# quan-dao/practical-collab-perception

Hardware: AMD Instinct MI355X
Metric: frames/sec (60k-pt cloud, 6 agents) (higher is better)
Workload: dtype f32

## Files before the change

### include/pcp_hip.h

```cpp
#ifndef PCP_HIP_H
#define PCP_HIP_H

#include <stddef.h>
#include <stdint.h>

#ifdef __cplusplus
extern "C" {
#endif

#define PCP_ABI_VERSION 1

enum {
  PCP_OK = 0,
  PCP_ERR_ARG = 1,
  PCP_ERR_WORKSPACE = 2,
  PCP_ERR_LAUNCH = 3,
  PCP_ERR_UNSUPPORTED = 4
};

int pcp_abi_version(void);
const char *pcp_status_string(int status);

enum {
  PCP_OPT_PFN_CROWD = 0,
  PCP_OPT_PFN_CROWD_BLOCKS = 1,
  PCP_OPT_PFN_WPS = 2,
  PCP_OPT_WINO4C_NW = 3,
  PCP_OPT_MP_TH16_MIN = 4,
  PCP_OPT_MP_DIAG = 5,
  PCP_OPT_VOX_AGGREGATE = 6,
  PCP_OPT_CONV_S2_FORM = 7,
  PCP_OPT_GTS_PASTE_FORM = 8,
  PCP_OPT_COUNT = 9
};
int pcp_set_option(int32_t option, int64_t value);
int64_t pcp_get_option(int32_t option);

typedef struct {
  float min_x, min_y, min_z;
  float voxel_x, voxel_y, voxel_z;
  int32_t nx, ny;
  int32_t batch_size;
} pcp_grid_t;

#define PCP_VOX_COUNTERS 4

size_t pcp_voxelize_workspace_bytes(const pcp_grid_t *grid, int64_t max_points);

int pcp_voxelize(const float *points, int64_t n, int32_t row_stride, const pcp_grid_t *grid,
                 void *workspace, size_t workspace_bytes,
                 int32_t *voxel_coords, int64_t *unq_inv, int32_t *unq_cnt, int32_t *counters, void *stream);
int pcp_voxelize_cells_ready(const float *points, int64_t n, int32_t row_stride, const pcp_grid_t *grid,
                             void *workspace, size_t workspace_bytes,
                             int32_t *voxel_coords, int32_t *unq_cnt, int32_t *counters, void *stream);

int pcp_voxelize_sort_pillar_rows(const pcp_grid_t *grid, void *workspace, int64_t n, void *stream);
int pcp_voxelize_row_order(const pcp_grid_t *grid, const void *workspace, int64_t n, int32_t *order, int32_t *cursor_scratch,
                           void *stream);

int pcp_pfn_scatter(const float *points, int64_t n, int32_t row_stride, int32_t num_raw, const pcp_grid_t *grid,
                    const void *workspace, const float *w0, const float *b0, const float *w1, const float *b1,
                    float *pillar_features, float *canvas, void *stream);

#define PCP_ROWS_CELLS_READY 1
#define PCP_ROWS_BUCKET_ORDER 2
size_t pcp_pillarise_rows_workspace_bytes(const pcp_grid_t *grid, int64_t max_points, int32_t num_raw);
int pcp_pillarise_rows(const float *points, int64_t n, int32_t row_stride, int32_t num_raw, const pcp_grid_t *grid,
                       void *workspace, size_t workspace_bytes, int32_t *voxel_coords, int64_t *unq_inv, int32_t *unq_cnt,
                       int32_t *counters, int32_t flags, void *stream);
int pcp_pfn_rows(const pcp_grid_t *grid, const void *workspace, int64_t n, int32_t num_raw, const float *w0, const float *b0,
                 const float *w1, const float *b1, float *pillar_features, float *canvas, void *stream);
int pcp_pillar_index_export(const pcp_grid_t *grid, const void *workspace, int64_t n, int32_t num_raw, int32_t *voxel_coords,
                            int32_t *row_rank, int32_t *slot_rank, int32_t *slot_canvas_row, int32_t *counters, void *stream);

#define PCP_PFN_ABSOLUTE_XYZ 1u
#define PCP_PFN_WITH_DISTANCE 2u
int pcp_pfn_features(const float *points, int64_t n, int32_t row_stride, int32_t num_raw, uint32_t flags, const pcp_grid_t *grid,
                     const void *vox_workspace, int32_t fw, float *fbuf, int32_t *slot_pillar, void *stream);
int pcp_pfn_cat_pillar_max(const float *y, int32_t ld_y, const float *pillar_max, int32_t ld_max, const int32_t *slot_pillar, int64_t rows,
                           int32_t c, float *out, int32_t ld_out, void *stream);

int pcp_canvas_clear(const pcp_grid_t *grid, const void *workspace, int64_t n, float *canvas, void *stream);
int pcp_fill_zero(void *ptr, size_t bytes, void *stream);

typedef struct {
  int32_t batch, in_h, in_w;
// ... 72 lines not shown
  int32_t batch, h, w, ld;
  int32_t num_class;
  int32_t ch_center, ch_z, ch_dim, ch_rot, ch_hm;
  int32_t k;
  float stride;
  float voxel_x, voxel_y, min_x, min_y;
  float limit[6];
  int32_t use_score_thresh;
  float score_thresh;
  int32_t activated;
} pcp_decode_t;

size_t pcp_decode_workspace_bytes(const pcp_decode_t *desc);
int pcp_centerhead_decode(const pcp_decode_t *desc, const float *head, void *workspace, size_t workspace_bytes,
                          float *boxes, float *scores, int32_t *labels, int32_t *cell, int32_t *count, void *stream);

#define PCP_DET_MAX_HEADS 8
typedef struct {
  const float *boxes;
  const float *scores;
  const int32_t *labels;
  const int32_t *keep;
  const int32_t *keep_count;
  const int32_t *class_map;
  int32_t k, keep_max;
} pcp_det_head_t;
int pcp_gather_detections(const pcp_det_head_t *heads, int32_t n_heads, int32_t batch, int32_t out_max, float *out_boxes,
                          float *out_scores, int64_t *out_labels, int32_t *out_count, void *stream);

size_t pcp_nms_workspace_bytes(int32_t n_max, int32_t batch);
int pcp_nms_rotated(const float *boxes, const float *scores, int32_t batch, int32_t n_max, const int32_t *n_dev,
                    float thresh, int32_t pre_max, int32_t post_max, void *workspace, size_t workspace_bytes,
                    int32_t *keep, int32_t *keep_count, void *stream);
int pcp_nms_normal(const float *boxes, const float *scores, int32_t batch, int32_t n_max, const int32_t *n_dev,
                   float thresh, int32_t pre_max, int32_t post_max, void *workspace, size_t workspace_bytes,
                   int32_t *keep, int32_t *keep_count, void *stream);
int pcp_boxes_bev_pairwise(const float *a, int32_t na, const float *b, int32_t nb, int32_t mode, float *out,
                           void *stream);

int pcp_warp_nearest(const float *src, float *dst, int32_t h, int32_t w, int32_t c, int32_t ld_src, int32_t ld_dst,
                     const float *theta_host, int32_t accumulate, void *stream);
int pcp_warp_nearest_batch(const float *const *src_host, float *const *dst_host, const float *theta_host, int32_t n_jobs, int32_t h,
                           int32_t w, int32_t c, int32_t ld_src, int32_t ld_dst, int32_t accumulate, void *stream);
int pcp_warp_nearest_batch_dev(const float *const *src_host, float *const *dst_host, const float *theta_dev, int32_t n_jobs, int32_t h,
                               int32_t w, int32_t c, int32_t ld_src, int32_t ld_dst, int32_t accumulate, void *stream);
int pcp_softmax_fuse(const float *const *maps_host, int32_t n_agents, const float *weights, int32_t ld_w, int64_t pixels,
                     int32_t c, int32_t ld_map, int32_t ld_out, float *out, void *stream);
int pcp_disco_weight_fuse(const float *const *maps_host, int32_t n_maps, int32_t c, int32_t ld_map, int64_t pixels,
                          const float *w1, const float *b1, const float *w2, const float *b2, const float *w3, const float *b3,
                          float *out, int32_t ld_out, float *logits, int32_t ld_w, void *stream);
int pcp_disco_weight_fuse_live(const float *const *maps_host, int32_t n_maps, int32_t c, int32_t ld_map, int64_t pixels,
                               const float *w1, const float *b1, const float *w2, const float *b2, const float *w3, const float *b3,
                               float *out, int32_t ld_out, const int32_t *live_index_host, const int32_t *live, void *stream);


int pcp_bev_sample_bilinear(const float *bev, int32_t batch, int32_t h, int32_t w, int32_t c, int32_t ld_bev,
                            const float *points, int64_t n, int32_t row_stride, float min_x, float min_y, float pix_x,
                            float pix_y, const uint8_t *row_mask, float *out, int32_t ld_out, void *stream);
int pcp_hunter_point_head(const float *bev, int32_t batch, int32_t h, int32_t w, int32_t c, int32_t ld_bev,
                          const float *points, int64_t n, int32_t row_stride, float min_x, float min_y, float pix_x,
                          float pix_y, const float *w1, const float *b1, const float *w2, const float *b2, const float *wh,
                          const float *bh, int32_t hidden, int32_t n_out, float *pf, int32_t ld_pf, float *head,
                          void *stream);
int pcp_hunter_point_head_ex(const float *bev, int32_t batch, int32_t h, int32_t w, int32_t c, int32_t ld_bev, float *points, int64_t n,
                             int32_t row_stride, float min_x, float min_y, float pix_x, float pix_y, const float *w1, const float *b1,
                             const float *w2, const float *b2, const float *wh, const float *bh, int32_t hidden, int32_t n_out, float *pf,
                             int32_t ld_pf, float *head, const int32_t *order, const int32_t *order_count, int32_t apply_flow,
                             float flow_thresh, uint8_t *dyn_mask, void *stream);
size_t pcp_bev_scatter_mean_workspace_bytes(int32_t batch, int32_t h, int32_t w, int64_t n);
int pcp_bev_scatter_mean(const float *points, int64_t n, int32_t row_stride, const float *feat, int32_t ld_feat,
                         int32_t c, int32_t batch, int32_t h, int32_t w, float min_x, float min_y, float pix_x,
                         float pix_y, void *workspace, size_t workspace_bytes, float *out, int32_t ld_out, void *stream);
int pcp_hunter_apply_flow(float *points, int64_t n, int32_t row_stride, const float *head, int32_t ld_head, float thresh,
                          uint8_t *row_mask, void *stream);

int pcp_select_transform_points(const float *points, int64_t n, int32_t row_stride, int32_t agent_col, float agent,
                                int32_t batch, const float *poses_host, const uint8_t *present_host, float *out,
                                int32_t out_batch_offset, void *stream);
int pcp_column_id_mask(const float *points, int64_t n, int32_t row_stride, int32_t col, uint64_t *out2, void *stream);
int pcp_column_id_counts(const float *points, int64_t n, int32_t row_stride, int32_t col, uint64_t *out66, void *stream);

int pcp_agent_frame_live(const float *points, int64_t n, int32_t row_stride, int32_t agent_col, int32_t batch, int32_t *live,
                         void *stream);
int pcp_zero_maps_unless(float *maps, int64_t map_elems, int32_t n_maps, const int32_t *flag_index_host, const int32_t *live,
                         void *stream);
size_t pcp_select_transform_compact_workspace_bytes(int64_t n, int32_t n_slots);
int pcp_select_transform_compact(const float *points, int64_t n, int32_t row_stride, int32_t agent_col, int32_t n_slots,
                                 const float *agents_host, int32_t batch, const float *poses_host, const uint8_t *present_host,
                                 float *out, int64_t out_rows, void *workspace, size_t workspace_bytes, int32_t *slot_start,
                                 const pcp_grid_t *vox_grid, void *vox_workspace, size_t vox_workspace_bytes, void *stream);
int pcp_select_transform_compact_dev(const float *points, int64_t n, int32_t row_stride, int32_t agent_col, int32_t n_slots,
                                     const float *agents_host, int32_t batch, const float *poses_dev, const uint8_t *present_dev,
                                     float *out, int64_t out_rows, void *workspace, size_t workspace_bytes, int32_t *slot_start,
                                     const pcp_grid_t *vox_grid, void *vox_workspace, size_t vox_workspace_bytes, void *stream);

int pcp_points_in_boxes(const float *boxes, int32_t batch, int32_t n_boxes, int32_t box_stride, const float *points, int32_t n_points,
                        int32_t point_stride, int32_t *box_idx, void *stream);
size_t pcp_hunter_foreground_workspace_bytes(int64_t n);
int pcp_hunter_foreground_rows(const float *points, int64_t n, int32_t row_stride, const float *head, int32_t ld_head, float thresh_bg,
                               void *workspace, size_t workspace_bytes, float *rows, int32_t *row_batch, int32_t *count, void *stream);
int pcp_modar_ingest(const float *modar, int32_t n_modar, const float *foreground, int32_t n_foreground, int32_t foreground_cols,
                     const double *target_se3_lidar_host, float max_sweep_idx, float *rows, void *stream);

size_t pcp_modar_ingest_batched_workspace_bytes(int32_t groups, int64_t max_foreground);
int pcp_modar_ingest_batched(const float *det_boxes, const float *det_scores, const int64_t *det_labels, const int32_t *det_count,
                             int32_t groups, int32_t det_max, const float *foreground, int32_t foreground_cols,
// ... 111 lines not shown
```

### practical-collab-perception_amd/csrc/abi.hip

```cpp
#include "pcp_common.h"

extern "C" int pcp_abi_version(void) { return PCP_ABI_VERSION; }

extern "C" const char *pcp_status_string(int status) {
  switch (status) {
    case PCP_OK: return "ok";
    case PCP_ERR_ARG: return "bad argument";
    case PCP_ERR_WORKSPACE: return "workspace too small";
    case PCP_ERR_LAUNCH: return "kernel launch failed";
    case PCP_ERR_UNSUPPORTED: return "unsupported shape for this build";
    default: return "unknown status";
  }
}

#include <atomic>

namespace {
std::atomic<long long> g_option[PCP_OPT_COUNT] = {{-1}, {-1}, {-1}, {-1}, {-1}, {-1}, {-1}, {-1}, {-1}};
static_assert(PCP_OPT_COUNT == 9, "one initialiser per option");
constexpr int MAX_DEVICES = 64;
std::atomic<int> g_cus[MAX_DEVICES];
}

extern "C" int pcp_set_option(int32_t option, int64_t value) {
  if (option < 0 || option >= PCP_OPT_COUNT) return PCP_ERR_ARG;
  g_option[option].store(value < 0 ? -1 : (long long)value, std::memory_order_relaxed);
  return PCP_OK;
}

extern "C" int64_t pcp_get_option(int32_t option) {
  if (option < 0 || option >= PCP_OPT_COUNT) return -1;
  return g_option[option].load(std::memory_order_relaxed);
}

long long pcp_option(int option, long long builtin) {
  const long long v = g_option[option].load(std::memory_order_relaxed);
  return v < 0 ? builtin : v;
}

int pcp_current_device_cus() {
  int dev = 0;
  if (hipGetDevice(&dev) != hipSuccess || dev < 0 || dev >= MAX_DEVICES) return 256;
  int v = g_cus[dev].load(std::memory_order_relaxed);
  if (v > 0) return v;
  if (hipDeviceGetAttribute(&v, hipDeviceAttributeMultiprocessorCount, dev) != hipSuccess || v <= 0) v = 256;
  g_cus[dev].store(v, std::memory_order_relaxed);
  return v;
}
```

### practical-collab-perception_amd/csrc/fusion.hip

```cpp
#include "pcp_common.h"

#pragma clang fp contract(off)

namespace {

struct Theta { float t[6]; };

__device__ __forceinline__ float base_coord(int i, int n) {
  if (n <= 1) return 0.f;
  float step = 2.0f / (float)(n - 1);
  float v = (i < n / 2) ? (-1.0f + step * (float)i) : (1.0f - step * (float)(n - 1 - i));
  return v * (float)(n - 1) / (float)n;
}

template <typename T> struct Map4;
template <> struct Map4<float> {
  static __device__ __forceinline__ float4 ld(const float *p) { return *reinterpret_cast<const float4 *>(p); }
  static __device__ __forceinline__ void st(float *p, const float4 &v) { *reinterpret_cast<float4 *>(p) = v; }
};
template <> struct Map4<__bf16> {
  typedef __bf16 b4 __attribute__((ext_vector_type(4)));
  static __device__ __forceinline__ float4 ld(const __bf16 *p) {
    const b4 v = *reinterpret_cast<const b4 *>(p);
    return make_float4((float)v[0], (float)v[1], (float)v[2], (float)v[3]);
  }
  static __device__ __forceinline__ void st(__bf16 *p, const float4 &v) {
    b4 o;
    o[0] = (__bf16)v.x; o[1] = (__bf16)v.y; o[2] = (__bf16)v.z; o[3] = (__bf16)v.w;
    *reinterpret_cast<b4 *>(p) = o;
  }
};

template <typename ST, typename DT>
__global__ void k_warp_nearest(const ST *__restrict__ src, DT *__restrict__ dst, int h, int w, int c4, int ld_src,
                               int ld_dst, Theta th, int accumulate) {
  long long t = (long long)blockIdx.x * blockDim.x + threadIdx.x;
  long long total = (long long)h * w * c4;
  if (t >= total) return;
  int q = (int)(t % c4);
  int pix = (int)(t / c4);
  int oy = pix / w, ox = pix % w;
  float xn = base_coord(ox, w), yn = base_coord(oy, h);
  float gx = xn * th.t[0] + yn * th.t[1] + th.t[2];
  float gy = xn * th.t[3] + yn * th.t[4] + th.t[5];
  float fx = (gx + 1.0f) * ((float)w / 2.0f) - 0.5f;
  float fy = (gy + 1.0f) * ((float)h / 2.0f) - 0.5f;
  float rx = nearbyintf(fx), ry = nearbyintf(fy);
  float4 v = make_float4(0.f, 0.f, 0.f, 0.f);
  if (rx >= 0.f && rx <= (float)(w - 1) && ry >= 0.f && ry <= (float)(h - 1)) {
    int sx = (int)rx, sy = (int)ry;
    v = Map4<ST>::ld(src + ((long long)sy * w + sx) * ld_src + q * 4);
  }
  DT *o = dst + (long long)pix * ld_dst + q * 4;
  if (accumulate) {
    float4 cur = Map4<DT>::ld(o);
    v.x += cur.x; v.y += cur.y; v.z += cur.z; v.w += cur.w;
  }
  Map4<DT>::st(o, v);
}

constexpr int WARP_MAX_JOBS = 32;
struct WarpJobs {
  const float *src[WARP_MAX_JOBS];
  float *dst[WARP_MAX_JOBS];
  Theta th[WARP_MAX_JOBS];
};

__global__ void k_warp_nearest_batch(WarpJobs jobs, int h, int w, int c4, int ld_src, int ld_dst, int accumulate, const float *__restrict__ theta_dev,
                                     int theta_first) {
  const int j = blockIdx.y;
  const float *__restrict__ src = jobs.src[j];
  float *__restrict__ dst = jobs.dst[j];
  Theta th = jobs.th[j];
  if (theta_dev) {
#pragma unroll
    for (int i = 0; i < 6; i++) th.t[i] = theta_dev[(theta_first + j) * 6 + i];
  }
  long long t = (long long)blockIdx.x * blockDim.x + threadIdx.x;
  long long total = (long long)h * w * c4;
  if (t >= total) return;
  int q = (int)(t % c4);
  int pix = (int)(t / c4);
  int oy = pix / w, ox = pix % w;
  float xn = base_coord(ox, w), yn = base_coord(oy, h);
  float gx = xn * th.t[0] + yn * th.t[1] + th.t[2];
  float gy = xn * th.t[3] + yn * th.t[4] + th.t[5];
  float fx = (gx + 1.0f) * ((float)w / 2.0f) - 0.5f;
  float fy = (gy + 1.0f) * ((float)h / 2.0f) - 0.5f;
  float rx = nearbyintf(fx), ry = nearbyintf(fy);
  float4 v = make_float4(0.f, 0.f, 0.f, 0.f);
  if (rx >= 0.f && rx <= (float)(w - 1) && ry >= 0.f && ry <= (float)(h - 1)) {
    int sx = (int)rx, sy = (int)ry;
    v = *reinterpret_cast<const float4 *>(src + ((long long)sy * w + sx) * ld_src + q * 4);
  }
  float4 *o = reinterpret_cast<float4 *>(dst + (long long)pix * ld_dst + q * 4);
  if (accumulate) {
    float4 cur = *o;
    v.x += cur.x; v.y += cur.y; v.z += cur.z; v.w += cur.w;
  }
  *o = v;
}

constexpr int MAX_AGENTS = 16;
struct MapPtrs { const float *p[MAX_AGENTS]; };
struct VMapPtrs { const void *p[MAX_AGENTS]; };

template <typename MT>
__global__ void k_softmax_fuse(VMapPtrs maps, int n_agents, const float *__restrict__ weights, int ld_w, long long pixels,
                               int c4, int ld_map, int ld_out, float *__restrict__ out) {
  long long t = (long long)blockIdx.x * blockDim.x + threadIdx.x;
  if (t >= pixels * c4) return;
  int q = (int)(t % c4);
  long long pix = t / c4;
  float wv[MAX_AGENTS];
  float mx = -INFINITY;
#pragma unroll
  for (int a = 0; a < MAX_AGENTS; a++)
    if (a < n_agents) {
      wv[a] = weights[pix * ld_w + a];
      mx = fmaxf(mx, wv[a]);
    }
  float den = 0.f;
#pragma unroll
  for (int a = 0; a < MAX_AGENTS; a++)
    if (a < n_agents) {
      wv[a] = expf(wv[a] - mx);
      den += wv[a];
    }
  float4 acc = make_float4(0.f, 0.f, 0.f, 0.f);
#pragma unroll
  for (int a = 0; a < MAX_AGENTS; a++)
    if (a < n_agents) {
      float s = wv[a] / den;
      float4 m = Map4<MT>::ld(reinterpret_cast<const MT *>(maps.p[a]) + pix * ld_map + q * 4);
      acc.x += m.x * s; acc.y += m.y * s; acc.z += m.z * s; acc.w += m.w * s;
    }
  *reinterpret_cast<float4 *>(out + pix * ld_out + q * 4) = acc;
}

}

extern "C" int pcp_warp_nearest(const float *src, float *dst, int32_t h, int32_t w, int32_t c, int32_t ld_src, int32_t ld_dst,
                                const float *theta_host, int32_t accumulate, void *stream_) {
  if (!src || !dst || !theta_host || h <= 0 || w <= 0 || c <= 0 || (c & 3) || (ld_src & 3) || (ld_dst & 3)) return PCP_ERR_ARG;
  if (src == dst) return PCP_ERR_ARG;
  Theta th;
  for (int i = 0; i < 6; i++) th.t[i] = theta_host[i];
// ... 53 lines not shown

extern "C" int pcp_mp_warp_nearest(const void *src, int32_t src_dtype, void *dst, int32_t dst_dtype, int32_t h, int32_t w, int32_t c,
                                   int32_t ld_src, int32_t ld_dst, const float *theta_host, int32_t accumulate, void *stream_) {
  if (!src || !dst || !theta_host || h <= 0 || w <= 0 || c <= 0 || (c & 3) || (ld_src & 3) || (ld_dst & 3)) return PCP_ERR_ARG;
  if (src == dst || (src_dtype | dst_dtype) & ~1) return PCP_ERR_ARG;
  Theta th;
  for (int i = 0; i < 6; i++) th.t[i] = theta_host[i];
  const long long total = (long long)h * w * (c / 4);
  const dim3 grid((unsigned)((total + 255) / 256));
  hipStream_t st = (hipStream_t)stream_;
#define PCP_WARP(ST, DT) hipLaunchKernelGGL((k_warp_nearest<ST, DT>), grid, dim3(256), 0, st, (const ST *)src, (DT *)dst, h, w, c / 4, ld_src, ld_dst, th, accumulate)
  if (src_dtype == 1) { if (dst_dtype == 1) PCP_WARP(__bf16, __bf16); else PCP_WARP(__bf16, float); }
  else { if (dst_dtype == 1) PCP_WARP(float, __bf16); else PCP_WARP(float, float); }
#undef PCP_WARP
  PCP_CHECK_LAUNCH();
  return PCP_OK;
}

extern "C" int pcp_mp_softmax_fuse(const void *const *maps_host, int32_t map_dtype, int32_t n_agents, const float *weights, int32_t ld_w,
                                   int64_t pixels, int32_t c, int32_t ld_map, int32_t ld_out, float *out, void *stream_) {
  if (!maps_host || !weights || !out || n_agents <= 0 || n_agents > MAX_AGENTS || pixels <= 0 || c <= 0 || (c & 3) ||
      (ld_map & 3) || (ld_out & 3) || ld_w < n_agents || (map_dtype & ~1))
    return PCP_ERR_ARG;
  VMapPtrs mp;
  for (int a = 0; a < MAX_AGENTS; a++) mp.p[a] = a < n_agents ? maps_host[a] : nullptr;
  const long long total = pixels * (c / 4);
  const dim3 grid((unsigned)((total + 255) / 256));
  if (map_dtype == 1)
    hipLaunchKernelGGL((k_softmax_fuse<__bf16>), grid, dim3(256), 0, (hipStream_t)stream_, mp, n_agents, weights, ld_w, (long long)pixels, c / 4,
                       ld_map, ld_out, out);
  else
    hipLaunchKernelGGL((k_softmax_fuse<float>), grid, dim3(256), 0, (hipStream_t)stream_, mp, n_agents, weights, ld_w, (long long)pixels, c / 4,
                       ld_map, ld_out, out);
  PCP_CHECK_LAUNCH();
  return PCP_OK;
}


namespace {

constexpr int WF_PX = 64;
constexpr int WF_C = 128;
constexpr int WF_H1 = 64, WF_H2 = 16;
constexpr int WF_H1_LD = 68;

struct WfParams {
  MapPtrs maps;
  int n_maps, ld_map, ld_out, ld_w;
  long long pixels;
  const float *w1, *b1, *w2, *b2, *w3, *b3;
  float *out, *logits;
  const int *live;
  int live_idx[MAX_AGENTS];
};

}

#pragma clang fp contract(on)
namespace {
}

namespace {

__global__ __launch_bounds__(256, 2) void k_weight_fuse(WfParams p) {
  __shared__ __attribute__((aligned(16))) float h1[WF_PX * WF_H1_LD];
  __shared__ float h2[WF_PX][WF_H2 + 1];
  __shared__ float lg[MAX_AGENTS][WF_PX];
  const int tid = threadIdx.x, lane = tid & 63;
  const int wave = __builtin_amdgcn_readfirstlane(tid >> 6);
  const int rt = wave >> 1, ct = wave & 1;
  const int r = lane & 31, h = lane >> 5;
  f32x4 wb[16];
  const float *w1_row = p.w1 + (long long)(ct * 32 + r) * (2 * WF_C) + 4 * h;
#pragma unroll
  for (int j = 0; j < 16; j++) wb[j] = *reinterpret_cast<const f32x4 *>(w1_row + WF_C + 8 * j);
  const float bias1 = p.b1[ct * 32 + r];
  const long long n_tiles = (p.pixels + WF_PX - 1) / WF_PX;
  for (long long tile = blockIdx.x; tile < n_tiles; tile += gridDim.x) {
    const long long px0 = tile * WF_PX;
    long long prow = px0 + rt * 32 + r;
    if (prow >= p.pixels) prow = p.pixels - 1;
    f32x16 acc_e;
#pragma unroll
    for (int e = 0; e < 16; e++) acc_e[e] = 0.f;
    {
      const float *src = p.maps.p[0] + prow * p.ld_map + 4 * h;
#pragma unroll
      for (int j = 0; j < 16; j++) {
        const f32x4 a = *reinterpret_cast<const f32x4 *>(src + 8 * j);
        const f32x4 w = *reinterpret_cast<const f32x4 *>(w1_row + 8 * j);
        acc_e = mfma32(a.x, w.x, acc_e);
        acc_e = mfma32(a.y, w.y, acc_e);
        acc_e = mfma32(a.z, w.z, acc_e);
        acc_e = mfma32(a.w, w.w, acc_e);
      }
    }
    for (int a_i = 0; a_i < p.n_maps; a_i++) {
      f32x16 acc = acc_e;
      const float *src = p.maps.p[a_i] + prow * p.ld_map + 4 * h;
#pragma unroll
      for (int j = 0; j < 16; j++) {
        const f32x4 a = *reinterpret_cast<const f32x4 *>(src + 8 * j);
        acc = mfma32(a.x, wb[j].x, acc);
        acc = mfma32(a.y, wb[j].y, acc);
        acc = mfma32(a.z, wb[j].z, acc);
        acc = mfma32(a.w, wb[j].w, acc);
      }
#pragma unroll
      for (int e = 0; e < 16; e++) {
        const int row = rt * 32 + (e & 3) + 8 * (e >> 2) + 4 * h;
        h1[row * WF_H1_LD + ct * 32 + r] = fmaxf(acc[e] + bias1, 0.f);
      }
      __syncthreads();
      {
        const int px = lane, og = wave;
        float o[4];
#pragma unroll
        for (int i = 0; i < 4; i++) o[i] = p.b2[og * 4 + i];
        const float *xr = &h1[px * WF_H1_LD];
#pragma unroll
        for (int k4 = 0; k4 < WF_H1 / 4; k4++) {
          const f32x4 x = *reinterpret_cast<const f32x4 *>(xr + 4 * k4);
#pragma unroll
          for (int i = 0; i < 4; i++) {
            const float *wr = p.w2 + (og * 4 + i) * WF_H1 + 4 * k4;
            o[i] = fmaf(wr[0], x.x, o[i]);
            o[i] = fmaf(wr[1], x.y, o[i]);
            o[i] = fmaf(wr[2], x.z, o[i]);
            o[i] = fmaf(wr[3], x.w, o[i]);
          }
        }
#pragma unroll
        for (int i = 0; i < 4; i++) h2[px][og * 4 + i] = fmaxf(o[i], 0.f);
      }
      __syncthreads();
      if (tid < WF_PX) {
        float l = p.b3[0];
#pragma unroll
        for (int k = 0; k < WF_H2; k++) l = fmaf(p.w3[k], h2[tid][k], l);
        l = fmaxf(l, 0.f);
        if (p.live && p.live_idx[a_i] >= 0 && p.live[p.live_idx[a_i]] == 0) l = -INFINITY;
        lg[a_i][tid] = l;
        if (p.logits && px0 + tid < p.pixels) p.logits[(px0 + tid) * p.ld_w + a_i] = l;
      }
    }
    __syncthreads();
    if (tid < WF_PX) {
      float mx = -INFINITY;
      for (int a_i = 0; a_i < p.n_maps; a_i++) mx = fmaxf(mx, lg[a_i][tid]);
      float den = 0.f;
      for (int a_i = 0; a_i < p.n_maps; a_i++) {
        const float e = expf(lg[a_i][tid] - mx);
        lg[a_i][tid] = e;
        den += e;
      }
      for (int a_i = 0; a_i < p.n_maps; a_i++) lg[a_i][tid] = lg[a_i][tid] / den;
    }
    __syncthreads();
    {
#pragma clang fp contract(off)
      constexpr int WF_Q = WF_PX * (WF_C / 4) / 256;
      float4 facc[WF_Q];
#pragma unroll
      for (int i = 0; i < WF_Q; i++) facc[i] = make_float4(0.f, 0.f, 0.f, 0.f);
      for (int a_i = 0; a_i < p.n_maps; a_i++) {
        float4 m[WF_Q];
        float sv[WF_Q];
#pragma unroll
        for (int i = 0; i < WF_Q; i++) {
          const int idx = i * 256 + tid;
          const int px = idx >> 5, q = idx & 31;
          long long pp = px0 + px;
          if (pp >= p.pixels) pp = p.pixels - 1;
          m[i] = *reinterpret_cast<const float4 *>(p.maps.p[a_i] + pp * p.ld_map + q * 4);
          sv[i] = lg[a_i][px];
        }
#pragma unroll
        for (int i = 0; i < WF_Q; i++) {
          facc[i].x += m[i].x * sv[i]; facc[i].y += m[i].y * sv[i]; facc[i].z += m[i].z * sv[i]; facc[i].w += m[i].w * sv[i];
        }
      }
#pragma unroll
      for (int i = 0; i < WF_Q; i++) {
        const int idx = i * 256 + tid;
        const int px = idx >> 5, q = idx & 31;
        if (px0 + px < p.pixels) *reinterpret_cast<float4 *>(p.out + (px0 + px) * p.ld_out + q * 4) = facc[i];
      }
    }
    __syncthreads();
  }
}

}

static int disco_weight_fuse_impl(const float *const *maps_host, int32_t n_maps, int32_t c, int32_t ld_map, int64_t pixels,
                                  const float *w1, const float *b1, const float *w2, const float *b2, const float *w3, const float *b3,
                                  float *out, int32_t ld_out, float *logits, int32_t ld_w, const int32_t *live_index_host, const int32_t *live,
                                  void *stream_) {
  if (!maps_host || !w1 || !b1 || !w2 || !b2 || !w3 || !b3 || !out || n_maps <= 0 || n_maps > MAX_AGENTS || pixels <= 0) return PCP_ERR_ARG;
  if (c != WF_C) return PCP_ERR_UNSUPPORTED;
  if ((ld_map & 3) || (ld_out & 3) || ld_map < c || ld_out < c || (logits && ld_w < n_maps)) return PCP_ERR_ARG;
  if ((((uintptr_t)w1) & 15) || (((uintptr_t)out) & 15)) return PCP_ERR_ARG;
  WfParams p;
  for (int a = 0; a < MAX_AGENTS; a++) {
    p.maps.p[a] = a < n_maps ? maps_host[a] : nullptr;
    if (a < n_maps && (!maps_host[a] || (((uintptr_t)maps_host[a]) & 15))) return PCP_ERR_ARG;
  }
  p.n_maps = n_maps; p.ld_map = ld_map; p.ld_out = ld_out; p.ld_w = ld_w; p.pixels = pixels;
  p.w1 = w1; p.b1 = b1; p.w2 = w2; p.b2 = b2; p.w3 = w3; p.b3 = b3; p.out = out; p.logits = logits;
  p.live = live_index_host ? live : nullptr;
  for (int a = 0; a < MAX_AGENTS; a++) p.live_idx[a] = (live_index_host && a < n_maps) ? live_index_host[a] : -1;
  const long long n_tiles = (pixels + WF_PX - 1) / WF_PX;
  const unsigned blocks = (unsigned)(n_tiles < 512 ? n_tiles : 512);
  hipLaunchKernelGGL(k_weight_fuse, dim3(blocks), dim3(256), 0, (hipStream_t)stream_, p);
  PCP_CHECK_LAUNCH();
  return PCP_OK;
}

extern "C" int pcp_disco_weight_fuse(const float *const *maps_host, int32_t n_maps, int32_t c, int32_t ld_map, int64_t pixels,
                                     const float *w1, const float *b1, const float *w2, const float *b2, const float *w3, const float *b3,
                                     float *out, int32_t ld_out, float *logits, int32_t ld_w, void *stream_) {
  return disco_weight_fuse_impl(maps_host, n_maps, c, ld_map, pixels, w1, b1, w2, b2, w3, b3, out, ld_out, logits, ld_w, nullptr, nullptr, stream_);
}

extern "C" int pcp_disco_weight_fuse_live(const float *const *maps_host, int32_t n_maps, int32_t c, int32_t ld_map, int64_t pixels,
                                          const float *w1, const float *b1, const float *w2, const float *b2, const float *w3, const float *b3,
                                          float *out, int32_t ld_out, const int32_t *live_index_host, const int32_t *live, void *stream_) {
  if (!live_index_host || !live) return PCP_ERR_ARG;
  return disco_weight_fuse_impl(maps_host, n_maps, c, ld_map, pixels, w1, b1, w2, b2, w3, b3, out, ld_out, nullptr, 0, live_index_host, live, stream_);
}
```

### practical-collab-perception_amd/pcdet/models/bev_layers/v2x_fusion_disco.py

```python
import os

import numpy as np
import torch
import torch.nn as nn

from pcp_amd import fusion_host, lib, ops

from ..convnet import pack_conv_module
from ..packed import PackedModule, train_tape


class PixelWeightedFusionSoftmax(nn.Module):

    def __init__(self, channel):
        super().__init__()
        self.conv1_1 = nn.Conv2d(channel * 2, 64, kernel_size=1, stride=1, padding=0)
        self.bn1_1 = nn.BatchNorm2d(64)
        self.conv1_2 = nn.Conv2d(64, 16, kernel_size=1, stride=1, padding=0)
        self.bn1_2 = nn.BatchNorm2d(16)
        self.conv1_4 = nn.Conv2d(16, 1, kernel_size=1, stride=1, padding=0)


def transform_bev_img(dst_se3_src, bev_in_src, pc_range_min, pix_size):
    assert bev_in_src.dim() == 3
# ... 36 lines not shown
                    d1=pack_conv_module(self.decompressor[3], None, relu=False),
                    wf=self._fold_weightor())

    fused_weightor = os.environ.get('PCP_DISCO_FUSED_WEIGHTOR', '1') != '0'

    def _fold_weightor(self):
        from ..convnet import _fold
        pw = self.pixel_weightor
        w1, b1 = _fold(pw.conv1_1, pw.bn1_1, 0)
        w2, b2 = _fold(pw.conv1_2, pw.bn1_2, 0)
        w3, b3 = _fold(pw.conv1_4, None, 0)
        f = lambda t: t.reshape(t.shape[0], -1).float().contiguous()
        return dict(w1=f(w1), b1=b1.float().contiguous(), w2=f(w2), b2=b2.float().contiguous(), w3=f(w3).reshape(-1).contiguous(),
                    b3=b3.float().reshape(1).contiguous())

    def _compress(self, pk, x_nhwc, out=None):
        h = pk['c0'].run(x_nhwc)
        if out is None:
            out = torch.empty(tuple(h.shape[:3]) + (pk['c1'].cout,), dtype=torch.float32, device=h.device)
        return pk['c1'].run(h, out=out)

    def compress_maps(self, bev_img_nchw):
        return self._compress(self.packed(), ops.as_nhwc(bev_img_nchw))

    def _weight(self, pk, ego, other, wbuf, col):
        h = ops.pointwise(ego, pk['w1'].w, pk['w1'].b, lib.PW_PLAIN, 2 * self.cc, 64, pk['w1'].cout_pad, relu=True, x2=other,
                          k_split=self.cc)
        h = pk['w2'].run(h)
        pk['w3'].run(h, out=wbuf, out_ch_off=col)

    def _forward_train(self, batch_dict):
        from ..train_path import FusionTrain
        from pcp_amd.train_layers import Act
        if getattr(self, '_pcp_train', None) is None:
            self._pcp_train = FusionTrain(self)
        self.invalidate_packed()
        out, loss = self._pcp_train.forward(Act(ops.as_nhwc(batch_dict['spatial_features_2d'])), batch_dict['bev_img'],
                                            batch_dict['metadata'], batch_dict.get('bev_img_early', None))
        if loss is not None:
            self.loss_dict['loss_distill'] = loss[0]
        batch_dict['spatial_features_2d'] = ops.nchw_view(out.t)
        train_tape(batch_dict).append(('v2x_mid_fusion', self._pcp_train.backward))
        return batch_dict

    @staticmethod
    def _warp_pairs(agent_order, metadata):
        return [(a, b) for a in agent_order for b, meta in enumerate(metadata) if a in meta['se3_from_ego']]

    def theta_array(self, metadata, agent_order, h, w):
        pairs = self._warp_pairs(agent_order, metadata)
        th = fusion_host.warp_thetas([metadata[b]['se3_from_ego'][a] for a, b in pairs], h, w, self.pc_min, self.pix_size)
        return np.asarray(th, dtype=np.float32).reshape(len(pairs), 6)

    def forward(self, batch_dict):
        if self.training:
            return self._forward_train(batch_dict)
        pk = self.packed()
        ego_in = ops.as_nhwc(batch_dict['spatial_features_2d'])
        self._last_map_hw = (int(ego_in.shape[1]), int(ego_in.shape[2]))
        B, H, W, _ = ego_in.shape
        agents = list(batch_dict['bev_img'].items())
        n_maps = 1 + len(agents)
        dev = ego_in.device
        stack = torch.empty((n_maps, B, H, W, self.cc), dtype=torch.float32, device=dev)
        self._compress(pk, ego_in, out=stack[0])
        fuse_now = self.fused_weightor and self.cc == 128 and n_maps <= 16 and pk['wf']['w1'].shape == (64, 2 * self.cc) \
            and pk['wf']['w2'].shape == (16, 64)
        wbuf = None
        if not fuse_now:
            wbuf = torch.zeros((B, H, W, max(4, (n_maps + 3) // 4 * 4)), dtype=torch.float32, device=dev)
            self._weight(pk, stack[0], stack[0], wbuf, 0)
        pre = batch_dict.get('bev_img_compressed', None)
        warps = []
        pairs = self._warp_pairs([agent_idx for agent_idx, _img in agents], batch_dict['metadata'])
        theta_list = fusion_host.warp_thetas([batch_dict['metadata'][b]['se3_from_ego'][a_] for a_, b in pairs], H, W, self.pc_min, self.pix_size)
        thetas = dict(zip(pairs, theta_list))
        for a, (agent_idx, bev_img) in enumerate(agents, start=1):
            comp = pre[agent_idx] if pre is not None else self._compress(pk, ops.as_nhwc(bev_img))
            for b_idx, meta in enumerate(batch_dict['metadata']):
                if agent_idx not in meta['se3_from_ego'] or b_idx >= comp.shape[0]:
                    stack[a, b_idx].zero_()
                    continue
                warps.append((comp[b_idx], stack[a, b_idx], thetas[(agent_idx, b_idx)]))
            if not fuse_now:
                ops.warp_nearest_batch(warps, self.cc)
                warps = []
                self._weight(pk, stack[0], stack[a], wbuf, a)
        table = batch_dict.get('_pcp_pose_table', None)
        theta_dev = None
        if table is not None and warps:
            assert fuse_now and len(warps) == len(pairs), 'graph mode: every listed (agent, frame) pair is warped in the one fused launch'
            theta_dev = table.slot('fusion.thetas', np.asarray([th for _s, _d, th in warps], dtype=np.float32).reshape(len(warps), 6))
        ops.warp_nearest_batch(warps, self.cc, theta_dev=theta_dev)
        live = batch_dict.get('_pcp_agent_live', None)
        if live is not None and agents:
            assert fuse_now, 'static agent discovery runs with the fused weightor'
            idx = [int(agent_idx) * B + b_idx if agent_idx in meta['se3_from_ego'] else -1
                   for agent_idx, _img in agents for b_idx, meta in enumerate(batch_dict['metadata'])]
            ops.zero_maps_unless(stack[1:].view(len(agents) * B, H, W, self.cc), idx, live)
        fused = torch.empty((B, H, W, self.cc), dtype=torch.float32, device=dev)
        if fuse_now:
            wf = pk['wf']
            live_index = None if live is None else [-1] + [int(agent_idx) * B for agent_idx, _img in agents]
            ops.disco_weight_fuse([stack[a] for a in range(n_maps)], wf['w1'], wf['b1'], wf['w2'], wf['b2'], wf['w3'], wf['b3'], self.cc, fused,
                                  live_index=live_index, live=live)
        else:
            ops.softmax_fuse([stack[a] for a in range(n_maps)], wbuf, self.cc, fused)
        out = pk['d1'].run(pk['d0'].run(fused), out=torch.empty((B, H, W, pk['d1'].cout), dtype=torch.float32, device=dev))
        batch_dict['spatial_features_2d'] = ops.nchw_view(out)
        return batch_dict
```

### practical-collab-perception_amd/pcp_amd/ops.py

```python
import ctypes

import torch

from . import lib as _lib
from .lib import Conv3x3, Decode, DecodeHead, DetHead, DetHeadExt, Grid, Pointwise, check
from .lib import (HARD_VOXEL_COUNTERS, HARD_VOXEL_MAX_BATCH, HARD_VOXEL_MAX_FEATURES, HARD_VOXEL_MAX_T, HARD_VOXEL_MIN_FEATURES,
                  MEAN_VFE_COUNTERS, MEAN_VFE_MAX_BATCH, MEAN_VFE_MAX_FEATURES, MEAN_VFE_MAX_NZ, MEAN_VFE_MIN_FEATURES, PFN_ABSOLUTE_XYZ,
                  PFN_WITH_DISTANCE, PILLAR_VFE_MAX_OUT, ROWS_BUCKET_ORDER, ROWS_CELLS_READY)


_RAW_STREAM = getattr(torch._C, '_cuda_getCurrentRawStream', None)
_CUR_DEVICE = getattr(torch._C, '_cuda_getDevice', None)


def current_stream_handle():
    if _RAW_STREAM is not None and _CUR_DEVICE is not None:
        return int(_RAW_STREAM(_CUR_DEVICE()))
    return int(torch.cuda.current_stream().cuda_stream)


def _stream():
    return ctypes.c_void_p(current_stream_handle())


# ... 590 lines not shown
    H, W, ld_s = jobs[0][0].shape
    ld_d = jobs[0][1].shape[2]
    for s_, d_, _t in jobs:
        assert tuple(s_.shape) == (H, W, ld_s) and tuple(d_.shape[:2]) == (H, W) and d_.shape[2] == ld_d
    n = len(jobs)
    src = (ctypes.c_void_p * n)(*[s_.data_ptr() for s_, _d, _t in jobs])
    dst = (ctypes.c_void_p * n)(*[d_.data_ptr() for _s, d_, _t in jobs])
    if theta_dev is not None:
        _need_cuda(theta_dev)
        assert theta_dev.dtype == torch.float32 and theta_dev.is_contiguous() and theta_dev.numel() == 6 * n
        check(L.pcp_warp_nearest_batch_dev(src, dst, _p(theta_dev), n, H, W, channels, ld_s, ld_d, 1 if accumulate else 0, _stream()),
              'pcp_warp_nearest_batch_dev')
        return
    th = (ctypes.c_float * (6 * n))(*[float(v) for _s, _d, t in jobs for v in t])
    check(L.pcp_warp_nearest_batch(src, dst, th, n, H, W, channels, ld_s, ld_d, 1 if accumulate else 0, _stream()), 'pcp_warp_nearest_batch')


def softmax_fuse(maps, weights, channels, out):
    _need_cuda(weights, out, *maps)
    _need_f32('pcp_softmax_fuse', weights, out, *maps)
    L = _lib.load()
    n = len(maps)
    arr = (ctypes.c_void_p * n)(*[m.data_ptr() for m in maps])
    pixels = weights.numel() // weights.shape[-1]
    check(L.pcp_softmax_fuse(arr, n, _p(weights), weights.shape[-1], pixels, channels, maps[0].shape[-1], out.shape[-1], _p(out),
                             _stream()), 'pcp_softmax_fuse')
    return out


def disco_weight_fuse(maps, w1, b1, w2, b2, w3, b3, channels, out, logits=None, live_index=None, live=None):
    _need_cuda(w1, b1, w2, b2, w3, b3, out, logits, live, *maps)
    _need_f32('pcp_disco_weight_fuse', out, logits, *maps)
    L = _lib.load()
    n = len(maps)
    arr = (ctypes.c_void_p * n)(*[m.data_ptr() for m in maps])
    ld_map = maps[0].shape[-1]
    pixels = maps[0].numel() // ld_map
    for m in maps:
        assert m.is_contiguous() and m.shape[-1] == ld_map and m.numel() // ld_map == pixels
    for t in (w1, b1, w2, b2, w3, b3):
        assert t.dtype == torch.float32 and t.is_contiguous()
    assert tuple(w1.shape) == (64, 2 * channels) and tuple(w2.shape) == (16, 64) and w3.numel() == 16 and b3.numel() == 1
    if live_index is not None:
        assert logits is None and live is not None and len(live_index) == n
        idx = (ctypes.c_int32 * n)(*[int(v) for v in live_index])
        check(L.pcp_disco_weight_fuse_live(arr, n, channels, ld_map, pixels, _p(w1), _p(b1), _p(w2), _p(b2), _p(w3), _p(b3), _p(out),
                                           out.shape[-1], idx, _p(live), _stream()), 'pcp_disco_weight_fuse_live')
        return out
    check(L.pcp_disco_weight_fuse(arr, n, channels, ld_map, pixels, _p(w1), _p(b1), _p(w2), _p(b2), _p(w3), _p(b3), _p(out), out.shape[-1],
                                  _p(logits), logits.shape[-1] if logits is not None else 0, _stream()), 'pcp_disco_weight_fuse')
    return out


def voxelize_sort_pillar_rows(vox):
    L = _lib.load()
    check(L.pcp_voxelize_sort_pillar_rows(ctypes.byref(vox.grid), _p(vox.workspace), vox.n, _stream()), 'pcp_voxelize_sort_pillar_rows')


def voxelize_row_order(vox):
    L = _lib.load()
    dev = vox.workspace.device
    order = torch.empty((max(vox.n, 1),), dtype=torch.int32, device=dev)
    cur = torch.empty((1,), dtype=torch.int32, device=dev)
    check(L.pcp_voxelize_row_order(ctypes.byref(vox.grid), _p(vox.workspace), vox.n, _p(order), _p(cur), _stream()), 'pcp_voxelize_row_order')
    return order


def hunter_point_head(bev, points, min_xy, pix_xy, w1, b1, w2, b2, wh, bh, channels, bev_ch_off=0, order=None, flow_thresh=None):
    _need_cuda(bev, points, w1, b1, w2, b2, wh, bh, order)
    L = _lib.load()
    B, H, W, ld_bev = bev.shape
    n, stride = points.shape
    pf = torch.empty((max(n, 1), channels), dtype=torch.float32, device=bev.device)
    head = torch.empty((max(n, 1), wh.shape[0]), dtype=torch.float32, device=bev.device)
    if order is not None or flow_thresh is not None:
        dyn = torch.zeros((max(n, 1),), dtype=torch.uint8, device=bev.device) if flow_thresh is not None else None
        check(L.pcp_hunter_point_head_ex(_chan_ptr(bev, bev_ch_off), B, H, W, channels, ld_bev, _p(points), n, stride, float(min_xy[0]),
                                         float(min_xy[1]), float(pix_xy[0]), float(pix_xy[1]), _p(w1), _p(b1), _p(w2), _p(b2), _p(wh),
                                         _p(bh), w1.shape[0], wh.shape[0], _p(pf), channels, _p(head), _p(order), ctypes.c_void_p(0),
                                         0 if flow_thresh is None else 1, 0.0 if flow_thresh is None else float(flow_thresh), _p(dyn),
                                         _stream()), 'pcp_hunter_point_head_ex')
        return (pf[:n], head[:n]) if flow_thresh is None else (pf[:n], head[:n], dyn[:n])
    check(L.pcp_hunter_point_head(_chan_ptr(bev, bev_ch_off), B, H, W, channels, ld_bev, _p(points), n, stride, float(min_xy[0]),
                                  float(min_xy[1]), float(pix_xy[0]), float(pix_xy[1]), _p(w1), _p(b1), _p(w2), _p(b2), _p(wh), _p(bh),
                                  w1.shape[0], wh.shape[0], _p(pf), channels, _p(head), _stream()), 'pcp_hunter_point_head')
    return pf[:n], head[:n]


def hunter_apply_flow(points, head, thresh):
    _need_cuda(points, head)
    L = _lib.load()
    n, stride = points.shape
    mask = torch.zeros((max(n, 1),), dtype=torch.uint8, device=points.device)
    check(L.pcp_hunter_apply_flow(_p(points), n, stride, _p(head), head.shape[1], float(thresh), _p(mask), _stream()),
          'pcp_hunter_apply_flow')
    return mask[:n]


def column_ids(points, col):
    import numpy as np
    _need_cuda(points)
    L = _lib.load()
    n, stride = points.shape
    out = torch.empty((2,), dtype=torch.int64, device=points.device)
    check(L.pcp_column_id_mask(_p(points), n, stride, col % stride, _p(out), _stream()), 'pcp_column_id_mask')
    mask, bad = [int(v) for v in out.cpu().tolist()]
# ... 495 lines not shown
```

Baseline: 402.6.

## Fuse nearest-neighbour BEV warp into DiSCo weight-fusion kernel via gather

Adds a gather variant of the DiSCo weight-fusion kernel that computes each agent's warped source pixel from the affine theta inside the kernel. Agent maps are then read directly from the compressed feature maps, with no separate warp pass into a stacked buffer. The intent is to remove the warp kernels' write and re-read traffic and the stack allocation. In exchange, loads become scattered gathers and a large parameter struct is passed per launch. The gathered path is selected by default through a new option when pair counts fit.

```diff
diff --git a/include/pcp_hip.h b/include/pcp_hip.h
--- a/include/pcp_hip.h
+++ b/include/pcp_hip.h
@@ -31,7 +31,8 @@
   PCP_OPT_VOX_AGGREGATE = 6,
   PCP_OPT_CONV_S2_FORM = 7,
   PCP_OPT_GTS_PASTE_FORM = 8,
-  PCP_OPT_COUNT = 9
+  PCP_OPT_DISCO_FUSE_FORM = 9,
+  PCP_OPT_COUNT = 10
 };
 int pcp_set_option(int32_t option, int64_t value);
 int64_t pcp_get_option(int32_t option);
@@ -210,6 +211,12 @@
 int pcp_disco_weight_fuse_live(const float *const *maps_host, int32_t n_maps, int32_t c, int32_t ld_map, int64_t pixels,
                                const float *w1, const float *b1, const float *w2, const float *b2, const float *w3, const float *b3,
                                float *out, int32_t ld_out, const int32_t *live_index_host, const int32_t *live, void *stream);
+int pcp_disco_weight_fuse_gather(const float *const *maps_host, const int32_t *map_frames_host, int32_t n_maps, int32_t frames, int32_t h,
+                                 int32_t w, int32_t c, int32_t ld_map, const float *theta_host, const float *theta_dev, int32_t theta_rows,
+                                 const int32_t *pair_row_host, const float *w1, const float *b1, const float *w2, const float *b2,
+                                 const float *w3, const float *b3, float *out, int32_t ld_out, const int32_t *live_index_host,
+                                 const int32_t *pair_live_host, const int32_t *live, void *stream);
+int32_t pcp_disco_fuse_form(int32_t n_maps, int32_t frames);
 
 
 int pcp_bev_sample_bilinear(const float *bev, int32_t batch, int32_t h, int32_t w, int32_t c, int32_t ld_bev,
diff --git a/practical-collab-perception_amd/csrc/abi.hip b/practical-collab-perception_amd/csrc/abi.hip
--- a/practical-collab-perception_amd/csrc/abi.hip
+++ b/practical-collab-perception_amd/csrc/abi.hip
@@ -16,8 +16,8 @@
 #include <atomic>
 
 namespace {
-std::atomic<long long> g_option[PCP_OPT_COUNT] = {{-1}, {-1}, {-1}, {-1}, {-1}, {-1}, {-1}, {-1}, {-1}};
-static_assert(PCP_OPT_COUNT == 9, "one initialiser per option");
+std::atomic<long long> g_option[PCP_OPT_COUNT] = {{-1}, {-1}, {-1}, {-1}, {-1}, {-1}, {-1}, {-1}, {-1}, {-1}};
+static_assert(PCP_OPT_COUNT == 10, "one initialiser per option");
 constexpr int MAX_DEVICES = 64;
 std::atomic<int> g_cus[MAX_DEVICES];
 }
diff --git a/practical-collab-perception_amd/csrc/fusion.hip b/practical-collab-perception_amd/csrc/fusion.hip
--- a/practical-collab-perception_amd/csrc/fusion.hip
+++ b/practical-collab-perception_amd/csrc/fusion.hip
@@ -11,6 +11,17 @@
   float step = 2.0f / (float)(n - 1);
   float v = (i < n / 2) ? (-1.0f + step * (float)i) : (1.0f - step * (float)(n - 1 - i));
   return v * (float)(n - 1) / (float)n;
+}
+
+__device__ __forceinline__ int warp_src_pixel(int ox, int oy, int h, int w, const Theta &th) {
+  float xn = base_coord(ox, w), yn = base_coord(oy, h);
+  float gx = xn * th.t[0] + yn * th.t[1] + th.t[2];
+  float gy = xn * th.t[3] + yn * th.t[4] + th.t[5];
+  float fx = (gx + 1.0f) * ((float)w / 2.0f) - 0.5f;
+  float fy = (gy + 1.0f) * ((float)h / 2.0f) - 0.5f;
+  float rx = nearbyintf(fx), ry = nearbyintf(fy);
+  if (rx >= 0.f && rx <= (float)(w - 1) && ry >= 0.f && ry <= (float)(h - 1)) return (int)ry * w + (int)rx;
+  return -1;
 }
 
 template <typename T> struct Map4;
@@ -40,17 +51,9 @@
   int q = (int)(t % c4);
   int pix = (int)(t / c4);
   int oy = pix / w, ox = pix % w;
-  float xn = base_coord(ox, w), yn = base_coord(oy, h);
-  float gx = xn * th.t[0] + yn * th.t[1] + th.t[2];
-  float gy = xn * th.t[3] + yn * th.t[4] + th.t[5];
-  float fx = (gx + 1.0f) * ((float)w / 2.0f) - 0.5f;
-  float fy = (gy + 1.0f) * ((float)h / 2.0f) - 0.5f;
-  float rx = nearbyintf(fx), ry = nearbyintf(fy);
+  const int sp = warp_src_pixel(ox, oy, h, w, th);
   float4 v = make_float4(0.f, 0.f, 0.f, 0.f);
-  if (rx >= 0.f && rx <= (float)(w - 1) && ry >= 0.f && ry <= (float)(h - 1)) {
-    int sx = (int)rx, sy = (int)ry;
-    v = Map4<ST>::ld(src + ((long long)sy * w + sx) * ld_src + q * 4);
-  }
+  if (sp >= 0) v = Map4<ST>::ld(src + (long long)sp * ld_src + q * 4);
   DT *o = dst + (long long)pix * ld_dst + q * 4;
   if (accumulate) {
     float4 cur = Map4<DT>::ld(o);
@@ -82,17 +85,9 @@
   int q = (int)(t % c4);
   int pix = (int)(t / c4);
   int oy = pix / w, ox = pix % w;
-  float xn = base_coord(ox, w), yn = base_coord(oy, h);
-  float gx = xn * th.t[0] + yn * th.t[1] + th.t[2];
-  float gy = xn * th.t[3] + yn * th.t[4] + th.t[5];
-  float fx = (gx + 1.0f) * ((float)w / 2.0f) - 0.5f;
-  float fy = (gy + 1.0f) * ((float)h / 2.0f) - 0.5f;
-  float rx = nearbyintf(fx), ry = nearbyintf(fy);
+  const int sp = warp_src_pixel(ox, oy, h, w, th);
   float4 v = make_float4(0.f, 0.f, 0.f, 0.f);
-  if (rx >= 0.f && rx <= (float)(w - 1) && ry >= 0.f && ry <= (float)(h - 1)) {
-    int sx = (int)rx, sy = (int)ry;
-    v = *reinterpret_cast<const float4 *>(src + ((long long)sy * w + sx) * ld_src + q * 4);
-  }
+  if (sp >= 0) v = *reinterpret_cast<const float4 *>(src + (long long)sp * ld_src + q * 4);
   float4 *o = reinterpret_cast<float4 *>(dst + (long long)pix * ld_dst + q * 4);
   if (accumulate) {
     float4 cur = *o;
@@ -252,6 +247,18 @@
   float *out, *logits;
   const int *live;
   int live_idx[MAX_AGENTS];
+  static constexpr bool gather = false;
+};
+
+constexpr int WF_MAX_PAIRS = 64;
+struct WfGatherParams : WfParams {
+  int h, w, frames;
+  int map_frames[MAX_AGENTS];
+  const float *theta_dev;
+  short row[WF_MAX_PAIRS];
+  int pair_live[WF_MAX_PAIRS];
+  Theta th[WF_MAX_PAIRS];
+  static constexpr bool gather = true;
 };
 
 }
@@ -262,10 +269,31 @@
 
 namespace {
 
-__global__ __launch_bounds__(256, 2) void k_weight_fuse(WfParams p) {
+__device__ __forceinline__ int wf_gather_row(const WfGatherParams &p, int a_i, int pp) {
+  if (a_i == 0) return pp;
+  const int hw = p.h * p.w;
+  const int b = pp / hw, pix = pp - b * hw;
+  const int pair = (a_i - 1) * p.frames + b;
+  const int row = p.row[pair];
+  bool there = row >= 0 && b < p.map_frames[a_i];
+  const int fl = p.pair_live[pair];
+  if (p.live && fl >= 0 && p.live[fl] == 0) there = false;
+  Theta th = p.th[pair];
+  if (p.theta_dev) {
+#pragma unroll
+    for (int i = 0; i < 6; i++) th.t[i] = p.theta_dev[(row < 0 ? 0 : row) * 6 + i];
+  }
+  const int sp = warp_src_pixel(pix % p.w, pix / p.w, p.h, p.w, th);
+  return (there && sp >= 0) ? b * hw + sp : -1;
+}
+
+template <typename P>
+__global__ __launch_bounds__(256, 2) void k_weight_fuse(P p) {
+  constexpr bool GATHER = P::gather;
   __shared__ __attribute__((aligned(16))) float h1[WF_PX * WF_H1_LD];
   __shared__ float h2[WF_PX][WF_H2 + 1];
   __shared__ float lg[MAX_AGENTS][WF_PX];
+  __shared__ int grow[GATHER ? MAX_AGENTS : 1][WF_PX];
   const int tid = threadIdx.x, lane = tid & 63;
   const int wave = __builtin_amdgcn_readfirstlane(tid >> 6);
   const int rt = wave >> 1, ct = wave & 1;
@@ -298,9 +326,18 @@
     for (int a_i = 0; a_i < p.n_maps; a_i++) {
       f32x16 acc = acc_e;
       const float *src = p.maps.p[a_i] + prow * p.ld_map + 4 * h;
+      bool zero_row = false;
+      if constexpr (GATHER) {
+        const int g = wf_gather_row(p, a_i, (int)prow);
+        if (ct == 0 && h == 0) grow[a_i][rt * 32 + r] = g;
+        zero_row = g < 0;
+        src = (zero_row ? p.maps.p[0] + prow * p.ld_map : p.maps.p[a_i] + (long long)g * p.ld_map) + 4 * h;
+      }
 #pragma unroll
       for (int j = 0; j < 16; j++) {
-        const f32x4 a = *reinterpret_cast<const f32x4 *>(src + 8 * j);
+        f32x4 a = *reinterpret_cast<const f32x4 *>(src + 8 * j);
+        if constexpr (GATHER)
+          if (zero_row) a = f32x4{0.f, 0.f, 0.f, 0.f};
         acc = mfma32(a.x, wb[j].x, acc);
         acc = mfma32(a.y, wb[j].y, acc);
         acc = mfma32(a.z, wb[j].z, acc);
@@ -372,7 +409,13 @@
           const int px = idx >> 5, q = idx & 31;
           long long pp = px0 + px;
           if (pp >= p.pixels) pp = p.pixels - 1;
-          m[i] = *reinterpret_cast<const float4 *>(p.maps.p[a_i] + pp * p.ld_map + q * 4);
+          if constexpr (GATHER) {
+            const int g = grow[a_i][px];
+            m[i] = *reinterpret_cast<const float4 *>((g < 0 ? p.maps.p[0] + pp * p.ld_map : p.maps.p[a_i] + (long long)g * p.ld_map) + q * 4);
+            if (g < 0) m[i] = make_float4(0.f, 0.f, 0.f, 0.f);
+          } else {
+            m[i] = *reinterpret_cast<const float4 *>(p.maps.p[a_i] + pp * p.ld_map + q * 4);
+          }
           sv[i] = lg[a_i][px];
         }
 #pragma unroll
@@ -412,7 +455,56 @@
   for (int a = 0; a < MAX_AGENTS; a++) p.live_idx[a] = (live_index_host && a < n_maps) ? live_index_host[a] : -1;
   const long long n_tiles = (pixels + WF_PX - 1) / WF_PX;
   const unsigned blocks = (unsigned)(n_tiles < 512 ? n_tiles : 512);
-  hipLaunchKernelGGL(k_weight_fuse, dim3(blocks), dim3(256), 0, (hipStream_t)stream_, p);
+  hipLaunchKernelGGL(k_weight_fuse<WfParams>, dim3(blocks), dim3(256), 0, (hipStream_t)stream_, p);
+  PCP_CHECK_LAUNCH();
+  return PCP_OK;
+}
+
+extern "C" int32_t pcp_disco_fuse_form(int32_t n_maps, int32_t frames) {
+  if (n_maps <= 0 || n_maps > MAX_AGENTS || frames <= 0 || (long long)(n_maps - 1) * frames > WF_MAX_PAIRS) return 1;
+  return pcp_option(PCP_OPT_DISCO_FUSE_FORM, 2) == 1 ? 1 : 2;
+}
+
+extern "C" int pcp_disco_weight_fuse_gather(const float *const *maps_host, const int32_t *map_frames_host, int32_t n_maps, int32_t frames, int32_t h,
+                                            int32_t w, int32_t c, int32_t ld_map, const float *theta_host, const float *theta_dev,
+                                            int32_t theta_rows, const int32_t *pair_row_host, const float *w1, const float *b1, const float *w2,
+                                            const float *b2, const float *w3, const float *b3, float *out, int32_t ld_out,
+                                            const int32_t *live_index_host, const int32_t *pair_live_host, const int32_t *live, void *stream_) {
+  if (!maps_host || !map_frames_host || !pair_row_host || !w1 || !b1 || !w2 || !b2 || !w3 || !b3 || !out) return PCP_ERR_ARG;
+  if (n_maps <= 0 || n_maps > MAX_AGENTS || frames <= 0 || h <= 0 || w <= 0 || theta_rows < 0) return PCP_ERR_ARG;
+  if (c != WF_C) return PCP_ERR_UNSUPPORTED;
+  const long long n_pairs = (long long)(n_maps - 1) * frames;
+  const long long pixels = (long long)frames * h * w;
+  if (n_pairs > WF_MAX_PAIRS || pixels > 0x7fffffffLL) return PCP_ERR_UNSUPPORTED;
+  if ((theta_host != nullptr) == (theta_dev != nullptr) && theta_rows > 0) return PCP_ERR_ARG;
+  if (theta_rows == 0 && (theta_host || theta_dev)) return PCP_ERR_ARG;
+  if ((ld_map & 3) || (ld_out & 3) || ld_map < c || ld_out < c) return PCP_ERR_ARG;
+  if ((((uintptr_t)w1) & 15) || (((uintptr_t)out) & 15)) return PCP_ERR_ARG;
+  if ((live_index_host || pair_live_host) && !live) return PCP_ERR_ARG;
+  WfGatherParams p;
+  for (int a = 0; a < MAX_AGENTS; a++) {
+    p.maps.p[a] = a < n_maps ? maps_host[a] : nullptr;
+    p.map_frames[a] = a < n_maps ? map_frames_host[a] : 0;
+    if (a < n_maps && (!maps_host[a] || (((uintptr_t)maps_host[a]) & 15) || map_frames_host[a] < 0 || map_frames_host[a] > frames)) return PCP_ERR_ARG;
+    if (a < n_maps && maps_host[a] == out) return PCP_ERR_ARG;
+    p.live_idx[a] = (live_index_host && a < n_maps) ? live_index_host[a] : -1;
+  }
+  if (map_frames_host[0] != frames) return PCP_ERR_ARG;
+  for (int i = 0; i < WF_MAX_PAIRS; i++) {
+    int row = i < n_pairs ? pair_row_host[i] : -1;
+    if (row >= theta_rows) return PCP_ERR_ARG;
+    if (row < 0) row = -1;
+    p.row[i] = (short)row;
+    p.pair_live[i] = (pair_live_host && i < n_pairs) ? pair_live_host[i] : -1;
+    for (int k = 0; k < 6; k++) p.th[i].t[k] = (theta_host && row >= 0) ? theta_host[row * 6 + k] : 0.f;
+  }
+  p.h = h; p.w = w; p.frames = frames; p.theta_dev = theta_dev;
+  p.n_maps = n_maps; p.ld_map = ld_map; p.ld_out = ld_out; p.ld_w = 0; p.pixels = pixels;
+  p.w1 = w1; p.b1 = b1; p.w2 = w2; p.b2 = b2; p.w3 = w3; p.b3 = b3; p.out = out; p.logits = nullptr;
+  p.live = (live_index_host || pair_live_host) ? live : nullptr;
+  const long long n_tiles = (pixels + WF_PX - 1) / WF_PX;
+  const unsigned blocks = (unsigned)(n_tiles < 512 ? n_tiles : 512);
+  hipLaunchKernelGGL(k_weight_fuse<WfGatherParams>, dim3(blocks), dim3(256), 0, (hipStream_t)stream_, p);
   PCP_CHECK_LAUNCH();
   return PCP_OK;
 }
diff --git a/practical-collab-perception_amd/pcdet/models/bev_layers/v2x_fusion_disco.py b/practical-collab-perception_amd/pcdet/models/bev_layers/v2x_fusion_disco.py
--- a/practical-collab-perception_amd/pcdet/models/bev_layers/v2x_fusion_disco.py
+++ b/practical-collab-perception_amd/pcdet/models/bev_layers/v2x_fusion_disco.py
@@ -112,6 +112,34 @@
         th = fusion_host.warp_thetas([metadata[b]['se3_from_ego'][a] for a, b in pairs], h, w, self.pc_min, self.pix_size)
         return np.asarray(th, dtype=np.float32).reshape(len(pairs), 6)
 
+    def _forward_gathered(self, batch_dict, pk, ego_in, agents):
+        B, H, W, _ = ego_in.shape
+        dev = ego_in.device
+        metadata = batch_dict['metadata']
+        ego = self._compress(pk, ego_in, out=torch.empty((B, H, W, self.cc), dtype=torch.float32, device=dev))
+        comps = [self._compress(pk, ops.as_nhwc(bev_img)) for _agent_idx, bev_img in agents]
+        pairs = self._warp_pairs([agent_idx for agent_idx, _img in agents], metadata)
+        thetas = fusion_host.warp_thetas([metadata[b]['se3_from_ego'][a_] for a_, b in pairs], H, W, self.pc_min, self.pix_size)
+        row_of = {pair: i for i, pair in enumerate(pairs)}
+        pair_rows = [[row_of.get((agent_idx, b), -1) for b in range(B)] for agent_idx, _img in agents]
+        table = batch_dict.get('_pcp_pose_table', None)
+        theta_dev = None
+        if table is not None and pairs:
+            theta_dev = table.slot('fusion.thetas', np.asarray(thetas, dtype=np.float32).reshape(len(pairs), 6))
+        live = batch_dict.get('_pcp_agent_live', None)
+        live_index = pair_live = None
+        if live is not None and agents:
+            pair_live = [[int(agent_idx) * B + b if row >= 0 else -1 for b, row in enumerate(rows)] for (agent_idx, _img), rows in zip(agents, pair_rows)]
+            live_index = [-1] + [int(agent_idx) * B for agent_idx, _img in agents]
+        fused = torch.empty((B, H, W, self.cc), dtype=torch.float32, device=dev)
+        wf = pk['wf']
+        ops.disco_weight_fuse_gather(ego, comps, pair_rows, wf['w1'], wf['b1'], wf['w2'], wf['b2'], wf['w3'], wf['b3'], self.cc, fused,
+                                     thetas=None if theta_dev is not None else thetas, theta_dev=theta_dev, live_index=live_index,
+                                     pair_live=pair_live, live=live)
+        out = pk['d1'].run(pk['d0'].run(fused), out=torch.empty((B, H, W, pk['d1'].cout), dtype=torch.float32, device=dev))
+        batch_dict['spatial_features_2d'] = ops.nchw_view(out)
+        return batch_dict
+
     def forward(self, batch_dict):
         if self.training:
             return self._forward_train(batch_dict)
@@ -122,10 +150,12 @@
         agents = list(batch_dict['bev_img'].items())
         n_maps = 1 + len(agents)
         dev = ego_in.device
+        fuse_now = self.fused_weightor and self.cc == 128 and n_maps <= 16 and pk['wf']['w1'].shape == (64, 2 * self.cc) \
+            and pk['wf']['w2'].shape == (16, 64)
+        if fuse_now and batch_dict.get('bev_img_compressed', None) is None and ops.disco_fuse_form(n_maps, B) == 2:
+            return self._forward_gathered(batch_dict, pk, ego_in, agents)
         stack = torch.empty((n_maps, B, H, W, self.cc), dtype=torch.float32, device=dev)
         self._compress(pk, ego_in, out=stack[0])
-        fuse_now = self.fused_weightor and self.cc == 128 and n_maps <= 16 and pk['wf']['w1'].shape == (64, 2 * self.cc) \
-            and pk['wf']['w2'].shape == (16, 64)
         wbuf = None
         if not fuse_now:
             wbuf = torch.zeros((B, H, W, max(4, (n_maps + 3) // 4 * 4)), dtype=torch.float32, device=dev)
diff --git a/practical-collab-perception_amd/pcp_amd/ops.py b/practical-collab-perception_amd/pcp_amd/ops.py
--- a/practical-collab-perception_amd/pcp_amd/ops.py
+++ b/practical-collab-perception_amd/pcp_amd/ops.py
@@ -666,6 +666,49 @@
     return out
 
 
+def disco_fuse_form(n_maps, frames):
+    return int(_lib.load().pcp_disco_fuse_form(int(n_maps), int(frames)))
+
+
+def disco_weight_fuse_gather(ego, agent_maps, pair_rows, w1, b1, w2, b2, w3, b3, channels, out, thetas=None, theta_dev=None, live_index=None,
+                             pair_live=None, live=None):
+    maps = [ego] + list(agent_maps)
+    _need_cuda(w1, b1, w2, b2, w3, b3, out, live, theta_dev, *maps)
+    _need_f32('pcp_disco_weight_fuse_gather', out, theta_dev, *maps)
+    L = _lib.load()
+    n = len(maps)
+    B, H, W, ld_map = ego.shape
+    for m in maps:
+        assert m.is_contiguous() and m.dim() == 4 and tuple(m.shape[1:]) == (H, W, ld_map) and m.shape[0] <= B
+    for t in (w1, b1, w2, b2, w3, b3):
+        assert t.dtype == torch.float32 and t.is_contiguous()
+    assert tuple(w1.shape) == (64, 2 * channels) and tuple(w2.shape) == (16, 64) and w3.numel() == 16 and b3.numel() == 1
+    assert out.is_contiguous() and out.numel() // out.shape[-1] == B * H * W
+    assert len(pair_rows) == n - 1 and all(len(r) == B for r in pair_rows)
+    assert (thetas is None) != (theta_dev is None)
+    if theta_dev is not None:
+        assert theta_dev.is_contiguous() and theta_dev.numel() % 6 == 0
+        rows, th = theta_dev.numel() // 6, None
+    else:
+        rows = len(thetas)
+        th = (ctypes.c_float * max(6 * rows, 1))(*[float(v) for t in thetas for v in t]) if rows else None
+    arr = (ctypes.c_void_p * n)(*[m.data_ptr() for m in maps])
+    frames = (ctypes.c_int32 * n)(*[int(m.shape[0]) for m in maps])
+    n_pairs = max((n - 1) * B, 1)
+    prow = (ctypes.c_int32 * n_pairs)(*[int(v) for r in pair_rows for v in r])
+    lidx = plive = None
+    if live_index is not None:
+        assert live is not None and len(live_index) == n
+        lidx = (ctypes.c_int32 * n)(*[int(v) for v in live_index])
+    if pair_live is not None:
+        assert live is not None and len(pair_live) == n - 1 and all(len(r) == B for r in pair_live)
+        plive = (ctypes.c_int32 * n_pairs)(*[int(v) for r in pair_live for v in r])
+    check(L.pcp_disco_weight_fuse_gather(arr, frames, n, B, H, W, channels, ld_map, th, _p(theta_dev) if rows else None, rows, prow, _p(w1), _p(b1),
+                                         _p(w2), _p(b2), _p(w3), _p(b3), _p(out), out.shape[-1], lidx, plive,
+                                         _p(live) if (lidx is not None or plive is not None) else None, _stream()), 'pcp_disco_weight_fuse_gather')
+    return out
+
+
 def voxelize_sort_pillar_rows(vox):
     L = _lib.load()
     check(L.pcp_voxelize_sort_pillar_rows(ctypes.byref(vox.grid), _p(vox.workspace), vox.n, _stream()), 'pcp_voxelize_sort_pillar_rows')
```

After: 399.6. No clear change (-0.8%).
